# HummaWhite/ReSTIR

Hardware: AMD Instinct MI355X
Metric: Mrays/s (1920x1080 ReSTIR-DI, 32 candidates, spatiotemporal reuse) (higher is better)
Workload: dtype f32

## Files before the change

include/restir_hip.h:

```cpp
#ifndef RESTIR_HIP_H
#define RESTIR_HIP_H

#include <stdint.h>

#ifdef __cplusplus
extern "C" {
#endif

#define RS_ERR_INVALID_ARGUMENT 10001
#define RS_ERR_UNSUPPORTED      10002
#define RS_ERR_INTERNAL         10003

typedef struct rs_material {
    int   type;
    float baseColor[3];
    float metallic;
    float roughness;
    float ior;
    int   baseColorMapId;
    int   metallicMapId;
    int   roughnessMapId;
    int   normalMapId;
} rs_material;

// ... 264 lines not shown
    int tuneCounted;
    int tuneRestart;
    int stream;
    int lastChains;
    int splitSlot, splitCall, splitMode;
    int shadowOnLibrary;
    int risForm;
    int tilesX, tilesY, fusedTilesY;
    int cut;
} rs_phase_a_plan;
int  rs_debug_phase_a_plan(const rs_phase_a_inputs* in, rs_phase_a_plan* out);
int  rs_restir_set_primary_cuts(rs_restir* r, int on);
int  rs_debug_set_primary_cut_cap(rs_restir* r, int records);
int  rs_debug_primary_cut_info(rs_restir* r, int* cells, int* cellsWithoutCut, unsigned long long* records, int* usedLastFrame, unsigned long long* builds);
int  rs_debug_primary_cut_missing(rs_restir* r, const rs_scene* scene, int cell, int n, const float* rays, unsigned long long out[4]);
int  rs_restir_set_primary_leaf_lists(rs_restir* r, int on);
int  rs_debug_set_primary_leaf_list_cap(rs_restir* r, int records);
int  rs_debug_primary_leaf_list_info(rs_restir* r, int* tiles, int* tilesWithoutList, unsigned long long* records, int* usedLastFrame, unsigned long long* builds);
int  rs_debug_primary_leaf_list_missing(rs_restir* r, const rs_scene* scene, int n, const float* rays, unsigned long long out[4]);
int  rs_debug_plan_primary_leaf_list(const rs_camera* cam, int x0, int y0, int bvhSize, const float* boundingBoxes, const int* const bvhNodes[6], int cap,
                                     int* order, int* count, int* positions);
int  rs_debug_plan_primary_cut(const rs_camera* cam, int x0, int y0, int w, int h, int bvhSize, const float* boundingBoxes, const int* const bvhNodes[6], int cap,
                               int* order, int* count, int* positions, int* links);
typedef struct rs_primary_cut_key {
    unsigned long long sceneId, geomEdits;
    rs_camera cam;
    int y0, y1;
    unsigned cap, listCap;
} rs_primary_cut_key;
#define RS_CUT_ARENA_NOTHING   0
#define RS_CUT_ARENA_NO_MEMORY 1
#define RS_CUT_ARENA_BUILT     2
typedef struct rs_primary_cut_slot { int keyValid, cuts, lists; rs_primary_cut_key key; } rs_primary_cut_slot;
typedef struct rs_primary_cut_sizes { int numCells; unsigned capacity; int numTiles; unsigned listCapacity; } rs_primary_cut_sizes;
int  rs_debug_plan_primary_cut_slot(int on, int capturing, rs_primary_cut_slot* slot, const rs_primary_cut_key* key, int tilesX, int tilesY,
                                    int* cutState, rs_primary_cut_sizes* sizes);
#ifndef RS_AUX_STREAMS
#define RS_AUX_STREAMS 3
#endif
#define RS_STREAM_CHOICES_KEPT 4
#define RS_STREAMS_HELD_NONE     0
#define RS_STREAMS_HELD_MEASURED 1
#define RS_STREAMS_HELD_PLAIN    2
#define RS_STREAMS_PENDING_NONE         0
#define RS_STREAMS_PENDING_AGAIN        1
#define RS_STREAMS_PENDING_AGAIN_FORGET 2
// ... 148 lines not shown
```

restir_amd/capi.py:

```python
import ctypes as C
import os

import numpy as np

from .ctypes_structs import Camera, Material, Reservoir, MATERIAL_DTYPE, RESERVOIR_DTYPE, INDIRECT_RESERVOIR_DTYPE, LIGHT_SAMPLE_DTYPE, copy_camera
from .ctypes_structs import GeometryEditLights, GeometryEditPlan, GeometryEditView
from .ctypes_structs import STREAM_CHOICES_KEPT, StreamChoice, StreamChoiceInputs, StreamChoicePlan, StreamChoices

_HERE = os.path.dirname(os.path.abspath(__file__))
LIB_PATH = os.environ.get("RESTIR_HIP_LIB") or os.path.join(_HERE, "librestir_hip.so")


class RestirHipError(RuntimeError):
    pass


RS_ERR_INVALID_ARGUMENT, RS_ERR_UNSUPPORTED = 10001, 10002

TRANSPORT_GROUP = C.CFUNCTYPE(C.c_int, C.c_void_p)
TRANSPORT_SEND = C.CFUNCTYPE(C.c_int, C.c_void_p, C.c_void_p, C.c_size_t, C.c_int, C.c_void_p)
TRANSPORT_RECV = C.CFUNCTYPE(C.c_int, C.c_void_p, C.c_void_p, C.c_size_t, C.c_int, C.c_void_p)


class Transport(C.Structure):
# ... 97 lines not shown


class PrimaryCutSlot(C.Structure):
    _fields_ = [("keyValid", C.c_int), ("cuts", C.c_int), ("lists", C.c_int), ("key", PrimaryCutKey)]


class PrimaryCutSizes(C.Structure):
    _fields_ = [("numCells", C.c_int), ("capacity", C.c_uint), ("numTiles", C.c_int), ("listCapacity", C.c_uint)]


CUT_ARENA_NOTHING, CUT_ARENA_NO_MEMORY, CUT_ARENA_BUILT = 0, 1, 2
STREAMS_HELD_NONE, STREAMS_HELD_MEASURED, STREAMS_HELD_PLAIN = 0, 1, 2
STREAMS_PENDING_NONE, STREAMS_PENDING_AGAIN, STREAMS_PENDING_AGAIN_FORGET = 0, 1, 2


EXPORTS = [
    "rs_last_error", "rs_context_create", "rs_context_destroy", "rs_context_set_current", "rs_init", "rs_set_stream", "rs_set_sync", "rs_set_side_stream", "rs_set_ris_table_pixels", "rs_set_internal_stream_priority", "rs_internal_streams_info", "rs_choose_internal_streams_again", "rs_prepare_streams", "rs_set_stream_plan", "rs_set_denoise_stream", "rs_join_denoise_stream", "rs_set_tile_split", "rs_debug_split_tiles", "rs_synchronize",
    "rs_build_bvh", "rs_build_light_table", "rs_build_alias_table", "rs_build_envmap_pdf", "rs_scene_build", "rs_scene_build_textured", "rs_scene_create",
    "rs_scene_host_desc", "rs_scene_set_sample_sequence", "rs_scene_set_emission", "rs_scene_set_materials", "rs_scene_set_texture", "rs_scene_set_triangles", "rs_scene_set_geometry", "rs_scene_set_motion_tracking", "rs_scene_advance_motion", "rs_scene_download_prev_vertices", "rs_refit_boxes", "rs_debug_scene_table", "rs_debug_scene_grid", "rs_debug_scene_emissive_grid", "rs_debug_grid_box", "rs_scene_destroy", "rs_camera_update", "rs_trace_closest", "rs_trace_closest_wave", "rs_scene_set_ordered_tree", "rs_ordered_bvh_host_check", "rs_trace_occlusion",
    "rs_gbuffer_create", "rs_gbuffer_destroy", "rs_gbuffer_render", "rs_gbuffer_render_rows", "rs_gbuffer_update",
    "rs_gbuffer_get_view", "rs_gbuffer_set_reuse", "rs_gbuffer_reuse_stats", "rs_gbuffer_invalidate", "rs_gbuffer_rows_bytes", "rs_gbuffer_rows_pack", "rs_gbuffer_rows_unpack", "rs_restir_init", "rs_restir_free", "rs_restir_reset", "rs_restir_direct",
    "rs_restir_phase_a", "rs_restir_phase_b", "rs_restir_end_frame", "rs_restir_launch_choice", "rs_restir_halo_bytes", "rs_restir_halo_pack",
    "rs_restir_halo_unpack", "rs_restir_rows_bytes", "rs_restir_rows_pack", "rs_restir_rows_unpack", "rs_restir_download", "rs_restir_upload", "rs_restir_set_light_tracking", "rs_restir_download_light_ids", "rs_restir_set_light_retargeting", "rs_restir_get_light_retargeting", "rs_restir_download_light_samples", "rs_debug_restir_retarget", "rs_debug_restir_retarget_launched", "rs_debug_restir_surface_wo", "rs_scene_light_moves", "rs_restir_light_rows_bytes", "rs_restir_light_rows_pack", "rs_restir_light_rows_unpack", "rs_restir_ray_count", "rs_restir_ray_total", "rs_restir_pass_times",
    "rs_restir_enable_timing", "rs_restir_spatial_times", "rs_restir_set_probe", "rs_restir_last_launch", "rs_debug_phase_a_plan", "rs_restir_set_primary_cuts", "rs_debug_set_primary_cut_cap", "rs_debug_primary_cut_info", "rs_debug_primary_cut_missing", "rs_restir_set_primary_leaf_lists", "rs_debug_set_primary_leaf_list_cap", "rs_debug_primary_leaf_list_info", "rs_debug_primary_leaf_list_missing", "rs_debug_plan_primary_leaf_list", "rs_debug_plan_primary_cut", "rs_debug_plan_primary_cut_slot", "rs_debug_plan_stream_choice", "rs_debug_plan_stream_switch", "rs_debug_restir_surface", "rs_pbo_register", "rs_pbo_map", "rs_pbo_unmap", "rs_pbo_unregister", "rs_save_image", "rs_save_image_jpg", "rs_write_png", "rs_write_jpg", "rs_debug_tap_estimate_error", "rs_debug_sqrt_of_uniform_mismatches", "rs_debug_sqrt_of_unit_floats_mismatches", "rs_debug_exact_ops_mismatches", "rs_debug_rng_step_mismatches", "rs_debug_rng_step_host_mismatches", "rs_debug_div_sigma_mismatches", "rs_path_trace_init", "rs_path_trace_free", "rs_path_trace_direct",
    "rs_path_trace", "rs_path_trace_indirect", "rs_restir_indirect", "rs_restir_download_indirect",
    "rs_svgf_create", "rs_svgf_destroy", "rs_svgf_filter", "rs_svgf_next_frame", "rs_svgf_get_view",
    "rs_copy_image_to_pbo", "rs_copy_image2_to_pbo", "rs_copy_imagef_to_pbo", "rs_copy_imagei_to_pbo", "rs_eaw_create", "rs_eaw_destroy", "rs_eaw_set_params", "rs_eaw_get_params", "rs_eaw_set_tiled", "rs_eaw_set_fused", "rs_svgf_set_params", "rs_svgf_get_params", "rs_svgf_set_tiled", "rs_svgf_set_fused", "rs_eaw_filter", "rs_eaw_positions_rows", "rs_eaw_level_rows", "rs_modulate_albedo",
    "rs_add_image", "rs_add_image3", "rs_comm_create_rccl", "rs_comm_create_rccl_lib", "rs_comm_create", "rs_comm_destroy", "rs_comm_self_exchange", "rs_strips_create", "rs_strips_destroy", "rs_strips_rows", "rs_strips_set_comm_stream", "rs_strips_set_gbuffer_halo", "rs_strips_set_light_tracking", "rs_strips_frame", "rs_strips_eaw_filter", "rs_strips_svgf_filter", "rs_strips_exchange_svgf_history", "rs_strips_exchange_history", "rs_strips_gather", "rs_strips_gather_begin", "rs_strips_gather_end", "rs_strips_enable_timing", "rs_strips_halo_wait_ms",
    "rs_scene_file_load", "rs_scene_file_get", "rs_scene_file_free", "rs_build_transformation_matrix", "rs_bake_instance",
    "rs_bake_matrix", "rs_scene_file_objects", "rs_scene_define_parts", "rs_scene_set_part_transforms", "rs_scene_parts_info", "rs_scene_download_part_rest", "rs_debug_scene_staged_bytes", "rs_debug_plan_geometry_edit",
]

_lib = None


def lib():
    global _lib
    if _lib is not None:
        return _lib
    try:
        import torch
    except ImportError:
        pass
    if not os.path.exists(LIB_PATH):
        raise RestirHipError(
            f"{LIB_PATH} is missing: build it with `make -C restir_amd/csrc` (or __graft_entry__.build()). "
            "There is no CPU fallback for the MI355X path.")
# ... 81 lines not shown
    L.rs_restir_launch_choice.argtypes = [vp, C.POINTER(ci)]
    L.rs_restir_halo_bytes.argtypes = [vp, ci]
    L.rs_restir_halo_bytes.restype = C.c_size_t
    L.rs_restir_halo_pack.argtypes = [vp, ci, ci, vp]
    L.rs_restir_halo_unpack.argtypes = [vp, ci, ci, vp]
    L.rs_restir_rows_bytes.argtypes = [vp, ci, ci]
    L.rs_restir_rows_bytes.restype = C.c_size_t
    L.rs_debug_tap_estimate_error.argtypes = [ci, C.POINTER(cf)]
    L.rs_restir_last_launch.argtypes = [vp, C.POINTER(ci), C.POINTER(ci)]
    L.rs_debug_phase_a_plan.argtypes = [C.POINTER(PhaseAInputs), C.POINTER(PhaseAPlan)]
    L.rs_debug_plan_geometry_edit.argtypes = [C.POINTER(GeometryEditView), C.c_char_p, ci, ci, vp, vp, vp, ci, C.POINTER(GeometryEditPlan), vp,
                                              C.POINTER(GeometryEditLights), vp, vp, vp]
    L.rs_restir_set_primary_cuts.argtypes = [vp, ci]
    L.rs_debug_set_primary_cut_cap.argtypes = [vp, ci]
    L.rs_debug_primary_cut_info.argtypes = [vp, C.POINTER(ci), C.POINTER(ci), C.POINTER(C.c_ulonglong), C.POINTER(ci), C.POINTER(C.c_ulonglong)]
    L.rs_debug_primary_cut_missing.argtypes = [vp, vp, ci, ci, vp, C.POINTER(C.c_ulonglong * 4)]
    L.rs_restir_set_primary_leaf_lists.argtypes = [vp, ci]
    L.rs_debug_set_primary_leaf_list_cap.argtypes = [vp, ci]
    L.rs_debug_primary_leaf_list_info.argtypes = [vp, C.POINTER(ci), C.POINTER(ci), C.POINTER(C.c_ulonglong), C.POINTER(ci), C.POINTER(C.c_ulonglong)]
    L.rs_debug_primary_leaf_list_missing.argtypes = [vp, vp, ci, vp, C.POINTER(C.c_ulonglong * 4)]
    L.rs_debug_plan_primary_leaf_list.argtypes = [vp, ci, ci, ci, vp, C.POINTER(vp * 6), ci, C.POINTER(ci), C.POINTER(ci), vp]
    L.rs_debug_plan_primary_cut.argtypes = [vp, ci, ci, ci, ci, ci, vp, C.POINTER(vp * 6), ci, C.POINTER(ci), C.POINTER(ci), vp, vp]
    L.rs_debug_plan_primary_cut_slot.argtypes = [ci, ci, C.POINTER(PrimaryCutSlot), C.POINTER(PrimaryCutKey), ci, ci, C.POINTER(ci), C.POINTER(PrimaryCutSizes)]
    L.rs_debug_plan_stream_choice.argtypes = [C.POINTER(StreamChoiceInputs), C.POINTER(StreamChoicePlan)]
    L.rs_debug_plan_stream_switch.argtypes = [C.POINTER(StreamChoices), ci, vp, ci, C.POINTER(StreamChoice), C.POINTER(ci)]
    L.rs_debug_restir_surface.argtypes = [vp, vp, vp, vp]
    L.rs_pbo_register.argtypes = [C.c_uint, C.POINTER(vp)]
    L.rs_pbo_map.argtypes = [vp, C.POINTER(vp), C.POINTER(C.c_size_t)]
    L.rs_pbo_unmap.argtypes = [vp]
    L.rs_pbo_unregister.argtypes = [vp]
    L.rs_save_image.argtypes = [C.c_char_p, vp, ci, ci, ci]
    L.rs_write_png.argtypes = [C.c_char_p, vp, ci, ci]
    L.rs_write_jpg.argtypes = [C.c_char_p, vp, ci, ci]
    L.rs_svgf_set_tiled.argtypes = [vp, ci]
    L.rs_svgf_set_fused.argtypes = [vp, ci]
    L.rs_save_image_jpg.argtypes = [C.c_char_p, vp, ci, ci, ci]
    L.rs_debug_sqrt_of_uniform_mismatches.argtypes = [C.POINTER(C.c_ulonglong)]
    L.rs_debug_sqrt_of_unit_floats_mismatches.argtypes = [C.POINTER(C.c_ulonglong)]
    L.rs_debug_exact_ops_mismatches.argtypes = [ci, C.c_uint, C.c_uint, ci, ci, C.POINTER(C.c_ulonglong)]
    L.rs_debug_div_sigma_mismatches.argtypes = [C.c_float, C.POINTER(C.c_ulonglong)]
    L.rs_debug_rng_step_mismatches.argtypes = [C.POINTER(C.c_ulonglong * 2)]
    L.rs_debug_rng_step_host_mismatches.argtypes = [C.c_uint, C.c_uint, C.POINTER(C.c_ulonglong * 2)]
    L.rs_scene_set_sample_sequence.argtypes = [vp, vp, ci, ci]
    L.rs_set_stream_plan.argtypes = [ci, ci, ci]
    L.rs_set_denoise_stream.argtypes = [ci]
    L.rs_join_denoise_stream.argtypes = []
# ... 226 lines not shown
    order, count = C.c_int(), C.c_int()
    pos = np.zeros(max(int(cap), 1), np.int32)
    check(lib().rs_debug_plan_primary_leaf_list(C.byref(cam), int(x0), int(y0), nodes.shape[1], _p(boxes), C.byref(arr), int(cap), C.byref(order), C.byref(count), _p(pos)))
    return order.value, count.value, pos[:min(count.value, int(cap))].copy()


def plan_primary_cut(cam, x0, y0, w, h, boxes, nodes, cap):
    boxes = np.ascontiguousarray(boxes, np.float32); nodes = np.ascontiguousarray(nodes, np.int32)
    arr = (C.c_void_p * 6)(*[nodes[i].ctypes.data for i in range(6)])
    order, count = C.c_int(), C.c_int()
    pos, links = np.zeros(max(int(cap), 1), np.int32), np.zeros(max(int(cap), 1), np.int32)
    check(lib().rs_debug_plan_primary_cut(C.byref(cam), int(x0), int(y0), int(w), int(h), nodes.shape[1], _p(boxes), C.byref(arr), int(cap),
                                          C.byref(order), C.byref(count), _p(pos), _p(links)))
    kept = min(count.value, int(cap))
    return order.value, count.value, pos[:kept].copy(), links[:kept if count.value <= int(cap) else 0].copy()


def plan_primary_cut_slot(slot, key, on=True, capturing=False, tiles=(1, 1)):
    state, sizes = C.c_int(), PrimaryCutSizes()
    check(lib().rs_debug_plan_primary_cut_slot(int(on), int(capturing), C.byref(slot), C.byref(key), int(tiles[0]), int(tiles[1]), C.byref(state), C.byref(sizes)))
    return state.value, sizes


def plan_stream_choice(priority_range, asked=2, caller_priority=None, times_us=None):
    i, o = StreamChoiceInputs(), StreamChoicePlan()
    i.least, i.greatest, i.asked = int(priority_range[0]), int(priority_range[1]), int(asked)
    i.callerHasStream, i.callerPriority = int(caller_priority is not None), int(caller_priority or 0)
    for lvl in range(3):
        for k in range(4):
            i.timesUs[lvl][k] = 1.0 if times_us is None else float(times_us[lvl][k])
    check(lib().rs_debug_plan_stream_choice(C.byref(i), C.byref(o)))
    return o


def plan_stream_switch(state, caller, level_key=2, forget=False):
    released, n = (StreamChoice * (STREAM_CHOICES_KEPT + 1))(), C.c_int()
    check(lib().rs_debug_plan_stream_switch(C.byref(state), int(forget), C.c_void_p(caller), int(level_key), released, C.byref(n)))
    return [released[k] for k in range(n.value)]


def build_bvh(vertices):
    v = np.ascontiguousarray(vertices, np.float32).reshape(-1)
    n = v.size // 9
    size = 2 * n - 1
    boxes = np.zeros((size, 6), np.float32)
    nodes = np.zeros((6, size, 3), np.int32)
# ... 510 lines not shown
        return a.value, b.value

    def set_primary_cuts(self, on=True):
        check(lib().rs_restir_set_primary_cuts(self.handle, 1 if on else 0))

    def set_primary_cut_cap(self, records):
        check(lib().rs_debug_set_primary_cut_cap(self.handle, records))

    def primary_cut_info(self):
        a, b, u = C.c_int(), C.c_int(), C.c_int()
        n, k = C.c_ulonglong(), C.c_ulonglong()
        check(lib().rs_debug_primary_cut_info(self.handle, C.byref(a), C.byref(b), C.byref(n), C.byref(u), C.byref(k)))
        return dict(cells=a.value, without_cut=b.value, records=n.value, used=bool(u.value), builds=k.value)

    def primary_cut_missing(self, scene, cell, rays):
        rays = np.ascontiguousarray(rays, np.float32).reshape(-1, 4)
        out = (C.c_ulonglong * 4)()
        check(lib().rs_debug_primary_cut_missing(self.handle, scene.handle, cell, len(rays), _p(rays), C.byref(out)))
        return dict(missing=out[0], passed=out[1], left_out=out[2], records=out[3])

    def set_primary_leaf_lists(self, on=True):
        check(lib().rs_restir_set_primary_leaf_lists(self.handle, 1 if on else 0))

    def set_primary_leaf_list_cap(self, records):
        check(lib().rs_debug_set_primary_leaf_list_cap(self.handle, records))

    def primary_leaf_list_info(self):
        a, b, u = C.c_int(), C.c_int(), C.c_int()
        n, k = C.c_ulonglong(), C.c_ulonglong()
        check(lib().rs_debug_primary_leaf_list_info(self.handle, C.byref(a), C.byref(b), C.byref(n), C.byref(u), C.byref(k)))
        return dict(tiles=a.value, without_list=b.value, records=n.value, used=bool(u.value), builds=k.value)

    def primary_leaf_list_missing(self, scene, rays):
        rays = np.ascontiguousarray(rays, np.float32).reshape(-1, 4)
        out = (C.c_ulonglong * 4)()
        check(lib().rs_debug_primary_leaf_list_missing(self.handle, scene.handle, len(rays), _p(rays), C.byref(out)))
        return dict(missing=out[0], passed=out[1], left_out=out[2])

    def surface(self):
        n = self.width * self.height
        a, b, c = np.zeros((n, 4), np.float32), np.zeros((n, 4), np.float32), np.zeros((n, 2), np.uint32)
        check(lib().rs_debug_restir_surface(self.handle, _p(a), _p(b), _p(c)))
        return a, b, c

    def surface_wo(self):
        out = np.zeros((self.width * self.height, 4), np.float32)
# ... 350 lines not shown
```

restir_amd/csrc/restir.hip:

```cpp
#include <cstdlib>
#include <cstring>

#include "rs_row_layouts.h"
#include "rs_light_history.h"
#include "rs_cuts.h"

using namespace rs;

namespace {

constexpr int kReservoirSize = 32;
constexpr int kHalo = RS_SPATIAL_HALO_ROWS;

constexpr int kDrawsPrimary = 4, kDrawsRis = kDrawsPrimary + 5 * 32;
constexpr unsigned kTemporalDrewBit = 1u << 29;
constexpr int kRaySlots = 1024;
template <bool TEX>
__device__ __forceinline__ int primary_store(const DevScene& s, const SurfPlanes& sp, int index, const Ray& ray, const Hit& h, unsigned rngWord) {
    int shaded = 0;
    int kind = kKindMiss, matId = 0, type = 0;
    f3 norm = splat(0.f), wo = splat(0.f), p = h.pos;
    float metallic = 0.f, roughness = 0.f;
    if (h.primId != kNullPrim) {
        matId = h.matId;
        norm = h.norm;
        const SurfMat m = TEX ? textured_material(s, h, norm) : plain_material(s, matId);
        type = m.type; metallic = m.metallic; roughness = m.roughness;
        if (type == 4) {
// ... 251 lines not shown
__device__ __forceinline__ float ld_stream(const float* p) { return __builtin_nontemporal_load(p); }
__device__ __forceinline__ int ld_stream(const int* p) { return __builtin_nontemporal_load(p); }
__device__ __forceinline__ f3 ld3_stream(const float* p) { return mk3(__builtin_nontemporal_load(p), __builtin_nontemporal_load(p + 1), __builtin_nontemporal_load(p + 2)); }
__device__ __forceinline__ void st_stream(float4* p, float x, float y, float z, float w) { __builtin_nontemporal_store(vf4{ x, y, z, w }, reinterpret_cast<vf4*>(p)); }

__device__ __forceinline__ void resv_store(const ResvPlanes& p, int i, const Resv& r) {
    st_stream(p.li + i, r.Li.x, r.Li.y, r.Li.z, r.dist);
    st_stream(p.wi + i, r.wi.x, r.wi.y, r.wi.z, 0.f);
    __builtin_nontemporal_store(r.W, p.w + i);
    __builtin_nontemporal_store(r.M, p.m + i);
}

__global__ void __launch_bounds__(256, RS_WALK_WAVES) k_shadow(DevScene s, SurfPlanes sp, int width, int y0, int y1, int tilesX) {
    RS_SETPRIO(RS_PRIO_WALK);
    int x, y;
    pixel_of_lane(tilesX, y0, x, y);
    const bool inside = x < width && y < y1;
    const int index = inside ? y * width + x : 0;
    const float4 pm = inside ? sp.posMat[index] : make_float4(0.f, 0.f, 0.f, 0.f);
    const bool shaded = inside && mk_kind(__float_as_int(pm.w)) == kKindShaded;
    float4 cl = make_float4(0.f, 0.f, 0.f, 0.f), cw = cl;
    if (shaded) { cl = sp.candLi[index]; cw = sp.candWi[index]; }
    const f3 pos = mk3(pm.x, pm.y, pm.z), wi = mk3(cw.x, cw.y, cw.z);
    const bool occluded = trace_occluded_wave(s, pos, pos + wi * cl.w, shaded);
    if (shaded && occluded) reinterpret_cast<float*>(sp.candWi + index)[3] = 0.f;
}

template <bool SOBOL, int LIGHTS>
__device__ __forceinline__ void temporal_body(const SurfPlanes& sp, const GBufView& g, const ResvPlanes& last, const ResvPlanes& cur, const TempPlanes& temp, const uint32_t* sampleSeq, int looper,
                                              int first, int reuse, int n0, int n1, unsigned long long* rayWork, unsigned long long* rayDone, const LightIds& ids,
                                              const LightRecs& recs) {
    constexpr bool TRACK = LIGHTS >= 1, RETARGET = LIGHTS == 2;
    RS_SETPRIO(RS_PRIO_STREAM);
    if (blockIdx.x == 0 && threadIdx.x < kRaySub) {
        const int k = threadIdx.x * kRayStride;
        rayDone[k] = rayWork[k];
        rayWork[k] = 0;
    }
    const int index = n0 + blockIdx.x * blockDim.x + threadIdx.x;
    if (index >= n1) return;
    const uint2 rm = sp.rngMat[index];
    const bool shaded = mk_kind((int)rm.y) == kKindShaded;
    const int gid = ld_stream(g.primId + index);
    const float gdepth = ld_stream(g.depth + index);
    if (!shaded) {
        if (reuse & 2) {
            reinterpret_cast<float2*>(temp.tap + index)[1] = make_float2(__int_as_float(gid), gdepth);
            if (TRACK) {
// ... 406 lines not shown
    rs_dev_free(r->dRayCount);
    for (auto& perStream : r->split) for (auto& t : perStream) rs_tile_split_free(&t);
    rs_dev_free(r->indResv[0]); rs_dev_free(r->indResv[1]);
    rs_light_history_free(r->lights);
    rs_primary_cuts_destroy(r->cuts);
    for (auto& e : r->ev) if (e) (void)hipEventDestroy(e);
    for (auto& pair : r->spatialEv) for (hipEvent_t& e : pair) if (e) (void)hipEventDestroy(e);
    for (auto& e : r->surfFree) if (e) (void)hipEventDestroy(e);
    for (auto& e : r->tune.ev) if (e) (void)hipEventDestroy(e);
    if (r->auxFork) (void)hipEventDestroy(r->auxFork);
    if (r->auxDone) (void)hipEventDestroy(r->auxDone);
    delete r;
    return 0;
}

int rs_restir_init(int width, int height, rs_restir** out) {
    if (!out || width <= 0 || height <= 0) return rs_fail(RS_ERR_INVALID_ARGUMENT, "rs_restir_init: bad size");
    *out = nullptr;
    rs_restir* r = new rs_restir();
    r->ctx = rs_ctx();
    rs_ctx_scope scope(r->ctx);
    r->width = width; r->height = height;
    rs_primary_cuts_init(r->cuts);
    const size_t n = (size_t)width * height;
    int e = 0;
    if (!e) e = alloc_planes(r->cur, n);
    if (!e) e = alloc_planes(r->last, n);
    if (!e) e = rs_dev_alloc(&r->temp.li, n);
    if (!e) e = rs_dev_alloc(&r->temp.wi, n);
    if (!e) e = rs_dev_alloc(&r->temp.tap, n);
    if (!e) e = rs_check_hip(hipMemset(r->temp.li, 0, n * 16), "memset");
    if (!e) e = rs_check_hip(hipMemset(r->temp.wi, 0, n * 16), "memset");
    if (!e) e = rs_check_hip(hipMemset(r->temp.tap, 0, n * 16), "memset");
    for (auto& f : r->surf) {
        if (!e) e = rs_dev_alloc(&f.posKind, n);
        if (!e) e = rs_dev_alloc(&f.norm, n);
        if (!e) e = rs_dev_alloc(&f.wo, n);
        if (!e) e = rs_dev_alloc(&f.rngMat, n);
        if (!e) e = rs_dev_alloc(&f.candLi, n);
        if (!e) e = rs_dev_alloc(&f.candWi, n);
        if (!e) e = rs_check_hip(hipMemset(f.rngMat, 0, n * 8), "memset");
    }
    for (auto& ev : r->surfFree) if (!e) e = rs_check_hip(hipEventCreateWithFlags(&ev, hipEventDisableTiming), "hipEventCreate");
    for (auto& ev : r->tune.ev) if (!e) e = rs_check_hip(hipEventCreate(&ev), "hipEventCreate");
    if (!e) e = rs_check_hip(hipEventCreateWithFlags(&r->auxFork, hipEventDisableTiming), "hipEventCreate");
    if (!e) e = rs_check_hip(hipEventCreateWithFlags(&r->auxDone, hipEventDisableTiming), "hipEventCreate");
// ... 8 lines not shown

int rs_restir_reset(rs_restir* r) {
    RS_SCOPE(r);
    if (!r) return rs_fail(RS_ERR_INVALID_ARGUMENT, "rs_restir_reset: null");
    r->firstFrame = true;
    return 0;
}

int rs_restir_enable_timing(rs_restir* r, int enable) {
    RS_SCOPE(r);
    if (!r) return rs_fail(RS_ERR_INVALID_ARGUMENT, "rs_restir_enable_timing: null");
    r->timing = enable == 2 ? 2 : (enable != 0 ? 1 : 0);
    if (r->timing == 2) {
        for (auto& pair : r->spatialEv) for (hipEvent_t& e : pair) if (!e) RS_HIP(hipEventCreate(&e));
        r->spatialNext = 0;
    }
    return 0;
}

int rs_restir_set_probe(rs_restir* r, int enable) {
    RS_SCOPE(r);
    if (!r) return rs_fail(RS_ERR_INVALID_ARGUMENT, "rs_restir_set_probe: null");
    r->probe = enable != 0;
    return 0;
}

int rs_restir_spatial_times(rs_restir* r, float* ms, int capacity, int* count) {
    RS_SCOPE(r);
    if (!r || !ms || !count || capacity < 0) return rs_fail(RS_ERR_INVALID_ARGUMENT, "rs_restir_spatial_times: bad argument");
    *count = 0;
    if (r->timing != 2) return rs_fail(RS_ERR_INVALID_ARGUMENT, "rs_restir_spatial_times: rs_restir_enable_timing(r, 2) is not in force");
    RS_HIP(hipStreamSynchronize(rs_stream()));
    int n = r->spatialNext < rs_restir::kSpatialRing ? r->spatialNext : rs_restir::kSpatialRing;
    if (n > capacity) n = capacity;
    for (int i = 0; i < n; i++) {
        const int slot = (r->spatialNext - n + i) % rs_restir::kSpatialRing;
        RS_HIP(hipEventElapsedTime(&ms[i], r->spatialEv[slot][0], r->spatialEv[slot][1]));
    }
    *count = n;
    return 0;
}

}

namespace {
int launch_ris(const rs_scene* scene, const SurfPlanes& sp, int W, int y0, int y1, int looper, bool sobol, hipStream_t st, int form, const rs_light_history& lights, int set) {
    const int npx = (y1 - y0) * W;
    const dim3 grid((npx + kRisThreads - 1) / kRisThreads);
    static const bool ldsAllowed = []{
        bool ok = true;
        for (int mode = 0; mode < 3; mode++) rs_dispatch_lights(mode, [&](auto LIGHTS) {
            for (const void* k : { reinterpret_cast<const void*>(&k_ris_alias_lds<true, LIGHTS()>), reinterpret_cast<const void*>(&k_ris_alias_lds<false, LIGHTS()>) })
                ok = hipFuncSetAttribute(k, hipFuncAttributeMaxDynamicSharedMemorySize, kRisAliasLdsLights * (int)sizeof(AliasRec)) == hipSuccess && ok;
        });
        (void)hipGetLastError();
        return ok; }();
    (void)ldsAllowed;
    rs_dispatch_lights(rs_light_mode(lights), [&](auto LIGHTS) {
        const RisWinners<LIGHTS()> win = rs_light_history_winners<LIGHTS()>(lights, set);
        if (form == RS_RIS_LDS)
            rs_dispatch([&](auto SOBOL) { hipLaunchKernelGGL((k_ris_lds<SOBOL(), LIGHTS()>), grid, dim3(kRisThreads), 0, st, scene->dev, sp, W, y0, y1, looper, win); }, sobol);
        else if (form == RS_RIS_ALIAS_LDS)
            rs_dispatch([&](auto SOBOL) { hipLaunchKernelGGL((k_ris_alias_lds<SOBOL(), LIGHTS()>), grid, dim3(kRisThreads), (size_t)scene->numLights * sizeof(AliasRec), st, scene->dev, sp, W, y0, y1, looper, win); }, sobol);
        else
            rs_dispatch([&](auto ENV, auto SOBOL) { hipLaunchKernelGGL((k_ris<ENV(), SOBOL(), LIGHTS()>), dim3((npx + 255) / 256), dim3(256), 0, st, scene->dev, sp, W, y0, y1, looper, win); },
                        scene->envMapTexId >= 0, sobol);
    });
    return 0;
}

int phase_a_impl(rs_restir* r, const rs_scene* scene, const rs_camera* cam, const rs_gbuffer* g, int looper, int reuse, int y0, int y1, bool last) {
    RS_TRY(check_frame_args(r, scene, cam, g));
    RS_TRY(rs_check_looper(scene, looper, "ReSTIRDirect"));
    const bool sobol = scene->dev.sampleSeq != nullptr;
    r->looper = looper;
    if (y0 < 0) y0 = 0;
    if (y1 > r->height) y1 = r->height;
    r->raySlot = (r->raySlot + 1) % kRaySlots;
    unsigned long long* rayCounter = r->dRayCount + (size_t)r->raySlot * kRaySub * kRayStride;
    unsigned long long* rayDone = rayCounter + (size_t)kRaySlots * kRaySub * kRayStride;
    const rs_context* plan = rs_stream_plan();
    const rs_gbuffer::Deferred& d = g->deferred;
    static const bool reusedThree = [] { const char* e = std::getenv("RS_REUSE_CHAINS"); return !(e && std::atoi(e) == 2); }();
    const int W = r->width;
    rs_phase_a_inputs in{};
    in.async = r->timing != 1 && rs_aux_stream(1) != nullptr;
    in.chainStreams = plan->chainStreams; in.smallChains = plan->smallChains; in.shadowOnMain = plan->shadowOnMain;
    in.fuseMode = rs_fuse_mode();
    in.denoiseStream = rs_ctx()->denoiseMode == 1;
    in.chainsInFlight = rs_chains_in_flight();
    in.reusedThree = reusedThree;
// ... 52 lines not shown
        RS_TRY(rs_tile_split_prepare(hints, ((((long long)1 << 20 | d.y0) << 20 | d.y1) << 12 | tilesX) ^ ((long long)(y0 * 4099 + y1) << 44), tilesX * 4 * gTilesY, tilesX * gTilesY, p.splitMode, st, &ts, &helpers));
        rs_dispatch([&](auto TEX, auto SOBOL, auto MOTION) {
            if (ts.base) hipLaunchKernelGGL((k_gbuffer_primary_split<TEX(), SOBOL(), MOTION()>), dim3(helpers + tilesX * gTilesY), dim3(256), 0, st, scene->dev, cp, lp, gw, sp, looper, d.y0, d.y1, y0, y1, tilesX, rayCounter, ts);
            else hipLaunchKernelGGL((k_gbuffer_primary<TEX(), SOBOL(), MOTION()>), dim3(tilesX * gTilesY), dim3(256), 0, st, scene->dev, cp, lp, gw, sp, looper, d.y0, d.y1, y0, y1, tilesX, rayCounter);
        }, tex, sobol, scene->dev.prevVertices != nullptr);
        RS_HIP(hipEventRecord(g->doneEv, aux));
        g->pending = true;
    }
    else {
        TileSplit ts; int helpers = 0;
        RS_TRY(rs_tile_split_prepare(hints, (((long long)y0 << 20 | y1) << 12 | tilesX), tilesX * 4 * tilesY, tilesX * tilesY, p.splitMode, st, &ts, &helpers));
        PrimaryCuts cuts{};
        if (p.cut == 2) RS_TRY(rs_primary_cuts_view(r->cuts, st, &cuts));
        rs_dispatch([&](auto TEX, auto SOBOL) {
            if (ts.base) hipLaunchKernelGGL((k_primary_split<TEX(), SOBOL()>), dim3(helpers + tilesX * tilesY), dim3(256), 0, st, scene->dev, cp, sp, looper, y0, y1, tilesX, rayCounter, ts, cuts);
            else hipLaunchKernelGGL((k_primary<TEX(), SOBOL()>), dim3(tilesX * tilesY), dim3(256), 0, st, scene->dev, cp, sp, looper, y0, y1, tilesX, rayCounter, cuts);
        }, tex, sobol);
        if (p.cut == 2) RS_TRY(rs_primary_cuts_launched(r->cuts, aux ? 1 + p.stream : 0, st));
    }
    mark(r, 1);
    const int npx = (y1 - y0) * W;
    RS_TRY(launch_ris(scene, sp, W, y0, y1, looper, sobol, st, p.risForm, r->lights, r->surfSet));
    mark(r, 2);
    if (!p.shadowOnLibrary) hipLaunchKernelGGL(k_shadow, dim3(tilesX * tilesY), dim3(256), 0, st, scene->dev, sp, W, y0, y1, tilesX);
    if (aux) {
        RS_TRY(rs_check_hip(hipGetLastError(), "ReSTIR Direct (primary / RIS / shadow rays)"));
        RS_HIP(hipEventRecord(r->auxDone, aux));
        RS_HIP(hipStreamWaitEvent(rs_stream(), r->auxDone, 0));
    }
    if (p.cut == 1) RS_TRY(rs_primary_cuts_build(r->cuts, scene, cp, y0, tilesX, tilesY, st));
    if (p.shadowOnLibrary) hipLaunchKernelGGL(k_shadow, dim3(tilesX * tilesY), dim3(256), 0, rs_stream(), scene->dev, sp, W, y0, y1, tilesX);
    RS_TRY(rs_gbuffer_join(g));
    LightIds ids; LightRecs recs;
    RS_TRY(rs_light_history_phase_a(r->lights, scene, r->surfSet, !r->firstFrame && (reuse & 1), sp, gbuf_view(g), r->last, y0, y1, tilesX, tilesY, rayCounter, &ids, &recs));
    rs_dispatch_lights(rs_light_mode(r->lights), [&](auto LIGHTS) {
        rs_dispatch([&](auto SOBOL) {
            hipLaunchKernelGGL((k_temporal<SOBOL(), LIGHTS()>), dim3((npx + 255) / 256), dim3(256), 0, rs_stream(), sp, gbuf_view(g), r->last, r->cur, r->temp,
                               scene->dev.sampleSeq, looper, r->firstFrame ? 1 : 0, reuse, y0 * W, y1 * W, rayCounter, rayDone, merge_lights<LIGHTS()>(ids, recs));
        }, sobol);
    });
    mark(r, 3);
    return last ? rs_after_launch("ReSTIR Direct (phase A)") : rs_check_hip(hipGetLastError(), "ReSTIR Direct (phase A)");
}

int phase_b_impl(rs_restir* r, const rs_scene* scene, const rs_camera* cam, const rs_gbuffer* g,
                 float* devDirectIllum, int iter, int reuse, int y0, int y1, bool last) {
    RS_TRY(check_frame_args(r, scene, cam, g));
    if (!devDirectIllum) return rs_fail(RS_ERR_INVALID_ARGUMENT, "ReSTIRDirect: null radiance buffer");
    if (y0 < 0) y0 = 0;
    if (y1 > r->height) y1 = r->height;
    if (y1 <= y0) return 0;
    const int tilesX = (r->width + kBTileW - 1) / kBTileW, tilesY = (y1 - y0 + kBTileH - 1) / kBTileH;
    const int numTiles = tilesX * tilesY;
    RS_TRY(rs_gbuffer_join(g));
// ... 44 lines not shown
    RS_SCOPE(r);
    return phase_b_impl(r, scene, cam, g, devDirectIllum, iter, reuse, y0, y1, true);
}

int rs_restir_last_launch(const rs_restir* r, int* fused, int* chains) {
    RS_SCOPE(r);
    if (!r || !fused || !chains) return rs_fail(RS_ERR_INVALID_ARGUMENT, "rs_restir_last_launch: null argument");
    *fused = r->lastFused; *chains = r->lastChains;
    return 0;
}

int rs_debug_restir_surface(rs_restir* r, float* posTag, float* normal, unsigned* rngTag) {
    RS_SCOPE(r);
    if (!r || !posTag || !normal || !rngTag) return rs_fail(RS_ERR_INVALID_ARGUMENT, "rs_debug_restir_surface: null argument");
    RS_TRY(rs_synchronize());
    const rs_restir::Surf& f = r->surf[(r->surfSet + rs_restir::kSurfSets - 1) % rs_restir::kSurfSets];
    const size_t n = (size_t)r->width * r->height;
    RS_HIP(hipMemcpy(posTag, f.posKind, n * 16, hipMemcpyDeviceToHost));
    RS_HIP(hipMemcpy(normal, f.norm, n * 16, hipMemcpyDeviceToHost));
    RS_HIP(hipMemcpy(rngTag, f.rngMat, n * 8, hipMemcpyDeviceToHost));
    return 0;
}

int rs_debug_restir_surface_wo(rs_restir* r, float* wo4) {
    RS_SCOPE(r);
    if (!r || !wo4) return rs_fail(RS_ERR_INVALID_ARGUMENT, "rs_debug_restir_surface_wo: null argument");
    RS_TRY(rs_synchronize());
    const rs_restir::Surf& f = r->surf[(r->surfSet + rs_restir::kSurfSets - 1) % rs_restir::kSurfSets];
    RS_HIP(hipMemcpy(wo4, f.wo, (size_t)r->width * r->height * 16, hipMemcpyDeviceToHost));
    return 0;
}

int rs_debug_phase_a_plan(const rs_phase_a_inputs* in, rs_phase_a_plan* out) {
    if (!in || !out) return rs_fail(RS_ERR_INVALID_ARGUMENT, "rs_debug_phase_a_plan: null argument");
    rs_plan_phase_a(*in, *out);
    return 0;
}

int rs_restir_launch_choice(const rs_restir* r, int* choice) {
    RS_SCOPE(r);
    if (!r || !choice) return rs_fail(RS_ERR_INVALID_ARGUMENT, "rs_restir_launch_choice: null argument");
    *choice = r->tune.reported();
    return 0;
}

int rs_restir_end_frame(rs_restir* r) {
// ... 207 lines not shown
```

restir_amd/csrc/rs_internal.h:

```cpp
#pragma once

#include <hip/hip_runtime.h>

#include <string>
#include <type_traits>
#ifndef RS_AUX_STREAMS
#define RS_AUX_STREAMS 3
#endif
#ifndef RS_SPLIT_SMALL_ROUNDS
#define RS_SPLIT_SMALL_ROUNDS 3
#endif
#include "rs_frame_plan.h"
#include "rs_cut_plan.h"
#include "rs_stream_choice.h"
#ifndef RS_GBUF_SETS
#define RS_GBUF_SETS (RS_AUX_STREAMS + 2)
#endif
#ifndef RS_SURF_SETS
#define RS_SURF_SETS (RS_AUX_STREAMS + 1)
#endif
#include <vector>

#include "rs_scene.h"
#include "rs_geometry_plan.h"
// ... 438 lines not shown
        uint2*  rngMat = nullptr;
        float4* candLi = nullptr;
        float4* candWi = nullptr;
    } surf[kSurfSets];
    int surfSet = 0, chain = 0, smallChain = 0;
    hipEvent_t surfFree[kSurfSets] = {};
    bool surfFreeValid[kSurfSets] = {};
    hipEvent_t auxFork = nullptr, auxDone = nullptr;
    int phaseACalls = 0;
    bool idleFrame = false;
    int idleStreak = 0;
    rs_fuse_tuner tune;
    int lastFused = -1, lastChains = 0;
    unsigned long long* dRayCount = nullptr;
    rs_tile_split split[1 + rs_context::kAux][3];
    int raySlot = 0;
    int timing = 0;
    hipEvent_t ev[5] = { nullptr, nullptr, nullptr, nullptr, nullptr };
    static constexpr int kSpatialRing = 256;
    hipEvent_t spatialEv[kSpatialRing][2] = {};
    int spatialNext = 0;
    bool probe = false;
    rs_light_history lights;
};

static_assert(rs_context::kAux >= 1 + rs_restir::kChains, "one auxiliary stream for GBuffer::render and one per chain");
static_assert(kPlanSmallChains == rs_context::kAux, "the plan's three chains are the context's auxiliary streams");

struct rs_eaw {
    rs_context* ctx = nullptr;
    int width = 0, height = 0, level = 0;
    float sigLumin = 64.f, sigNormal = .2f, sigDepth = 1.f;
    float* devTempImg = nullptr;
    float* devPos = nullptr;
    bool tiled = true;
    bool fused = true;
};

struct rs_svgf {
    rs_context* ctx = nullptr;
    int width = 0, height = 0, level = 0;
    float sigLumin = 4.f, sigNormal = 128.f, sigDepth = 1.f;
    float* devAccumColor[2] = { nullptr, nullptr };
    float* devAccumMoment[2] = { nullptr, nullptr };
    float* devVariance = nullptr;
    float* devTempColor = nullptr;
// ... 33 lines not shown
```

Before: 8276.

## Regroup shadow rays by length within each block before tracing occlusion

Adds a shadow-ray kernel that bins each tile's active shadow rays by length (relative to the scene extent) using a shared-memory histogram and prefix scan. Rays are compacted into LDS sorted longest-first, and each wave traces a coherent batch. Waves with no active rays exit early. The old kernel also now skips rays whose candidate weight is already zero. This targets wave divergence and idle lanes in the BVH occlusion walk, at the cost of extra LDS traffic, block-wide barriers and a scattered write-back of results. The feature is on by default.

```diff
diff --git a/include/restir_hip.h b/include/restir_hip.h
--- a/include/restir_hip.h
+++ b/include/restir_hip.h
@@ -310,6 +310,11 @@
                                      int* order, int* count, int* positions);
 int  rs_debug_plan_primary_cut(const rs_camera* cam, int x0, int y0, int w, int h, int bvhSize, const float* boundingBoxes, const int* const bvhNodes[6], int cap,
                                int* order, int* count, int* positions, int* links);
+int  rs_restir_set_shadow_regroup(rs_restir* r, int on);
+int  rs_debug_plan_shadow_regroup(int n, const float* lengths, const unsigned char* active, float binsOverExtent, const float* rootLo, const float* rootHi,
+                                  int* bins, int* first, int* count, float* binsOverExtentOut);
+int  rs_debug_shadow_pass(rs_restir* r, const rs_scene* scene, int y0, int y1, const float* posTag, const float* candLi, float* candWi, int* slots,
+                          float* binsOverExtent);
 typedef struct rs_primary_cut_key {
     unsigned long long sceneId, geomEdits;
     rs_camera cam;
diff --git a/restir_amd/capi.py b/restir_amd/capi.py
--- a/restir_amd/capi.py
+++ b/restir_amd/capi.py
@@ -143,7 +143,7 @@
     "rs_gbuffer_get_view", "rs_gbuffer_set_reuse", "rs_gbuffer_reuse_stats", "rs_gbuffer_invalidate", "rs_gbuffer_rows_bytes", "rs_gbuffer_rows_pack", "rs_gbuffer_rows_unpack", "rs_restir_init", "rs_restir_free", "rs_restir_reset", "rs_restir_direct",
     "rs_restir_phase_a", "rs_restir_phase_b", "rs_restir_end_frame", "rs_restir_launch_choice", "rs_restir_halo_bytes", "rs_restir_halo_pack",
     "rs_restir_halo_unpack", "rs_restir_rows_bytes", "rs_restir_rows_pack", "rs_restir_rows_unpack", "rs_restir_download", "rs_restir_upload", "rs_restir_set_light_tracking", "rs_restir_download_light_ids", "rs_restir_set_light_retargeting", "rs_restir_get_light_retargeting", "rs_restir_download_light_samples", "rs_debug_restir_retarget", "rs_debug_restir_retarget_launched", "rs_debug_restir_surface_wo", "rs_scene_light_moves", "rs_restir_light_rows_bytes", "rs_restir_light_rows_pack", "rs_restir_light_rows_unpack", "rs_restir_ray_count", "rs_restir_ray_total", "rs_restir_pass_times",
-    "rs_restir_enable_timing", "rs_restir_spatial_times", "rs_restir_set_probe", "rs_restir_last_launch", "rs_debug_phase_a_plan", "rs_restir_set_primary_cuts", "rs_debug_set_primary_cut_cap", "rs_debug_primary_cut_info", "rs_debug_primary_cut_missing", "rs_restir_set_primary_leaf_lists", "rs_debug_set_primary_leaf_list_cap", "rs_debug_primary_leaf_list_info", "rs_debug_primary_leaf_list_missing", "rs_debug_plan_primary_leaf_list", "rs_debug_plan_primary_cut", "rs_debug_plan_primary_cut_slot", "rs_debug_plan_stream_choice", "rs_debug_plan_stream_switch", "rs_debug_restir_surface", "rs_pbo_register", "rs_pbo_map", "rs_pbo_unmap", "rs_pbo_unregister", "rs_save_image", "rs_save_image_jpg", "rs_write_png", "rs_write_jpg", "rs_debug_tap_estimate_error", "rs_debug_sqrt_of_uniform_mismatches", "rs_debug_sqrt_of_unit_floats_mismatches", "rs_debug_exact_ops_mismatches", "rs_debug_rng_step_mismatches", "rs_debug_rng_step_host_mismatches", "rs_debug_div_sigma_mismatches", "rs_path_trace_init", "rs_path_trace_free", "rs_path_trace_direct",
+    "rs_restir_enable_timing", "rs_restir_spatial_times", "rs_restir_set_probe", "rs_restir_last_launch", "rs_debug_phase_a_plan", "rs_restir_set_primary_cuts", "rs_debug_set_primary_cut_cap", "rs_debug_primary_cut_info", "rs_debug_primary_cut_missing", "rs_restir_set_primary_leaf_lists", "rs_debug_set_primary_leaf_list_cap", "rs_debug_primary_leaf_list_info", "rs_debug_primary_leaf_list_missing", "rs_debug_plan_primary_leaf_list", "rs_debug_plan_primary_cut", "rs_debug_plan_primary_cut_slot", "rs_restir_set_shadow_regroup", "rs_debug_plan_shadow_regroup", "rs_debug_shadow_pass", "rs_debug_plan_stream_choice", "rs_debug_plan_stream_switch", "rs_debug_restir_surface", "rs_pbo_register", "rs_pbo_map", "rs_pbo_unmap", "rs_pbo_unregister", "rs_save_image", "rs_save_image_jpg", "rs_write_png", "rs_write_jpg", "rs_debug_tap_estimate_error", "rs_debug_sqrt_of_uniform_mismatches", "rs_debug_sqrt_of_unit_floats_mismatches", "rs_debug_exact_ops_mismatches", "rs_debug_rng_step_mismatches", "rs_debug_rng_step_host_mismatches", "rs_debug_div_sigma_mismatches", "rs_path_trace_init", "rs_path_trace_free", "rs_path_trace_direct",
     "rs_path_trace", "rs_path_trace_indirect", "rs_restir_indirect", "rs_restir_download_indirect",
     "rs_svgf_create", "rs_svgf_destroy", "rs_svgf_filter", "rs_svgf_next_frame", "rs_svgf_get_view",
     "rs_copy_image_to_pbo", "rs_copy_image2_to_pbo", "rs_copy_imagef_to_pbo", "rs_copy_imagei_to_pbo", "rs_eaw_create", "rs_eaw_destroy", "rs_eaw_set_params", "rs_eaw_get_params", "rs_eaw_set_tiled", "rs_eaw_set_fused", "rs_svgf_set_params", "rs_svgf_get_params", "rs_svgf_set_tiled", "rs_svgf_set_fused", "rs_eaw_filter", "rs_eaw_positions_rows", "rs_eaw_level_rows", "rs_modulate_albedo",
@@ -271,6 +271,10 @@
     L.rs_debug_plan_primary_leaf_list.argtypes = [vp, ci, ci, ci, vp, C.POINTER(vp * 6), ci, C.POINTER(ci), C.POINTER(ci), vp]
     L.rs_debug_plan_primary_cut.argtypes = [vp, ci, ci, ci, ci, ci, vp, C.POINTER(vp * 6), ci, C.POINTER(ci), C.POINTER(ci), vp, vp]
     L.rs_debug_plan_primary_cut_slot.argtypes = [ci, ci, C.POINTER(PrimaryCutSlot), C.POINTER(PrimaryCutKey), ci, ci, C.POINTER(ci), C.POINTER(PrimaryCutSizes)]
+    if hasattr(L, "rs_restir_set_shadow_regroup"):
+        L.rs_restir_set_shadow_regroup.argtypes = [vp, ci]
+        L.rs_debug_plan_shadow_regroup.argtypes = [ci, vp, vp, C.c_float, vp, vp, vp, vp, C.POINTER(ci), C.POINTER(C.c_float)]
+        L.rs_debug_shadow_pass.argtypes = [vp, vp, ci, ci, vp, vp, vp, vp, C.POINTER(C.c_float)]
     L.rs_debug_plan_stream_choice.argtypes = [C.POINTER(StreamChoiceInputs), C.POINTER(StreamChoicePlan)]
     L.rs_debug_plan_stream_switch.argtypes = [C.POINTER(StreamChoices), ci, vp, ci, C.POINTER(StreamChoice), C.POINTER(ci)]
     L.rs_debug_restir_surface.argtypes = [vp, vp, vp, vp]
@@ -543,6 +547,17 @@
     return state.value, sizes
 
 
+def plan_shadow_regroup(lengths, bins_over_extent=None, root=None, active=None, plan=False):
+    lengths = np.ascontiguousarray(lengths, np.float32).reshape(-1)
+    n = len(lengths)
+    bins, first, count, used = np.zeros(max(n, 1), np.int32), np.zeros(64, np.int32), C.c_int(), C.c_float()
+    act = None if active is None else np.ascontiguousarray(np.asarray(active) != 0, np.uint8)
+    lo, hi = (None, None) if root is None else (np.ascontiguousarray(root[0], np.float32), np.ascontiguousarray(root[1], np.float32))
+    check(lib().rs_debug_plan_shadow_regroup(n, _p(lengths), None if act is None else _p(act), float(bins_over_extent or 0.0), None if lo is None else _p(lo),
+                                             None if hi is None else _p(hi), _p(bins), _p(first) if plan else None, C.byref(count) if plan else None, C.byref(used)))
+    return (bins[:n], used.value, first, count.value) if plan else (bins[:n], used.value)
+
+
 def plan_stream_choice(priority_range, asked=2, caller_priority=None, times_us=None):
     i, o = StreamChoiceInputs(), StreamChoicePlan()
     i.least, i.greatest, i.asked = int(priority_range[0]), int(priority_range[1]), int(asked)
@@ -1099,6 +1114,17 @@
     def set_primary_leaf_lists(self, on=True):
         check(lib().rs_restir_set_primary_leaf_lists(self.handle, 1 if on else 0))
 
+    def set_shadow_regroup(self, on=True):
+        check(lib().rs_restir_set_shadow_regroup(self.handle, 1 if on else 0))
+
+    def shadow_pass(self, scene, pos_tag, cand_li, cand_wi, rows=None):
+        n = self.width * self.height
+        y0, y1 = rows or (0, self.height)
+        a, b = np.ascontiguousarray(pos_tag, np.float32).reshape(n, 4), np.ascontiguousarray(cand_li, np.float32).reshape(n, 4)
+        w, slots, k = np.array(cand_wi, np.float32).reshape(n, 4).copy(), np.zeros(n, np.int32), C.c_float()
+        check(lib().rs_debug_shadow_pass(self.handle, scene.handle, y0, y1, _p(a), _p(b), _p(w), _p(slots), C.byref(k)))
+        return w, slots, k.value
+
     def set_primary_leaf_list_cap(self, records):
         check(lib().rs_debug_set_primary_leaf_list_cap(self.handle, records))
 
diff --git a/restir_amd/csrc/restir.hip b/restir_amd/csrc/restir.hip
--- a/restir_amd/csrc/restir.hip
+++ b/restir_amd/csrc/restir.hip
@@ -4,6 +4,7 @@
 #include "rs_row_layouts.h"
 #include "rs_light_history.h"
 #include "rs_cuts.h"
+#include "rs_shadow_regroup.h"
 
 using namespace rs;
 
@@ -301,8 +302,48 @@
     float4 cl = make_float4(0.f, 0.f, 0.f, 0.f), cw = cl;
     if (shaded) { cl = sp.candLi[index]; cw = sp.candWi[index]; }
     const f3 pos = mk3(pm.x, pm.y, pm.z), wi = mk3(cw.x, cw.y, cw.z);
-    const bool occluded = trace_occluded_wave(s, pos, pos + wi * cl.w, shaded);
-    if (shaded && occluded) reinterpret_cast<float*>(sp.candWi + index)[3] = 0.f;
+    const bool walks = shaded && __float_as_uint(cw.w) != 0u;
+    const bool occluded = trace_occluded_wave(s, pos, pos + wi * cl.w, walks);
+    if (walks && occluded) reinterpret_cast<float*>(sp.candWi + index)[3] = 0.f;
+}
+
+__global__ void __launch_bounds__(kShadowRegroupRays, RS_WALK_WAVES) k_shadow_regroup(DevScene s, SurfPlanes sp, int width, int y0, int y1, int tilesX, float binsOverExtent, int* slotsOut) {
+    __shared__ float4 sRay[2 * kShadowRegroupRays];
+    __shared__ int sHist[kShadowBins];
+    RS_SETPRIO(RS_PRIO_WALK);
+    int x, y;
+    const int lane = pixel_of_lane(tilesX, y0, x, y);
+    if (threadIdx.x < kShadowBins) sHist[threadIdx.x] = 0;
+    const bool inside = x < width && y < y1;
+    const int index = inside ? y * width + x : 0;
+    const float4 pm = inside ? sp.posMat[index] : make_float4(0.f, 0.f, 0.f, 0.f);
+    const bool shaded = inside && mk_kind(__float_as_int(pm.w)) == kKindShaded;
+    float4 cl = make_float4(0.f, 0.f, 0.f, 0.f), cw = cl;
+    if (shaded) { cl = sp.candLi[index]; cw = sp.candWi[index]; }
+    const bool walks = shaded && __float_as_uint(cw.w) != 0u;
+    const int bin = shadow_bin(cl.w, binsOverExtent);
+    __syncthreads();
+    int rank = 0;
+    if (walks) rank = atomicAdd(&sHist[bin], 1);
+    __syncthreads();
+    int above = sHist[kShadowBins - 1 - lane];
+    for (int off = 1; off < 64; off <<= 1) { const int v = __shfl_up(above, off); above += lane >= off ? v : 0; }
+    const int count = __shfl(above, 63);
+    const int first = __shfl(above, bin < kShadowBins - 1 ? kShadowBins - 2 - bin : 0);
+    const int slot = (bin < kShadowBins - 1 ? first : 0) + rank;
+    if (walks) {
+        sRay[slot] = make_float4(pm.x, pm.y, pm.z, __int_as_float(index));
+        sRay[kShadowRegroupRays + slot] = make_float4(cw.x, cw.y, cw.z, cl.w);
+    }
+    if (slotsOut && inside) slotsOut[index] = walks ? slot : -1;
+    __syncthreads();
+    if ((int)(threadIdx.x & ~63u) >= count) return;
+    const bool mine = (int)threadIdx.x < count;
+    float4 a = make_float4(0.f, 0.f, 0.f, 0.f), b = a;
+    if (mine) { a = sRay[threadIdx.x]; b = sRay[kShadowRegroupRays + threadIdx.x]; }
+    const f3 pos = mk3(a.x, a.y, a.z), wi = mk3(b.x, b.y, b.z);
+    const bool occluded = trace_occluded_wave(s, pos, pos + wi * b.w, mine);
+    if (mine && occluded) reinterpret_cast<float*>(sp.candWi + __float_as_int(a.w))[3] = 0.f;
 }
 
 template <bool SOBOL, int LIGHTS>
@@ -755,6 +796,7 @@
     rs_ctx_scope scope(r->ctx);
     r->width = width; r->height = height;
     rs_primary_cuts_init(r->cuts);
+    if (const char* env = std::getenv("RS_SHADOW_REGROUP")) r->shadowRegroup = std::atoi(env) != 0;
     const size_t n = (size_t)width * height;
     int e = 0;
     if (!e) e = alloc_planes(r->cur, n);
@@ -809,6 +851,28 @@
     RS_SCOPE(r);
     if (!r) return rs_fail(RS_ERR_INVALID_ARGUMENT, "rs_restir_set_probe: null");
     r->probe = enable != 0;
+    return 0;
+}
+
+int rs_restir_set_shadow_regroup(rs_restir* r, int on) {
+    RS_SCOPE(r);
+    if (!r) return rs_fail(RS_ERR_INVALID_ARGUMENT, "rs_restir_set_shadow_regroup: null");
+    r->shadowRegroup = on != 0;
+    return 0;
+}
+
+int rs_debug_plan_shadow_regroup(int n, const float* lengths, const unsigned char* active, float binsOverExtent, const float* rootLo, const float* rootHi,
+                                 int* bins, int* first, int* count, float* binsOverExtentOut) {
+    if (n < 0 || (n > 0 && (!lengths || !bins)) || (!rootLo != !rootHi) || (!first != !count) || (first && n > kShadowRegroupRays))
+        return rs_fail(RS_ERR_INVALID_ARGUMENT, "rs_debug_plan_shadow_regroup: bad argument");
+    if (rootLo) binsOverExtent = shadow_bins_over_extent(rootLo, rootHi);
+    if (binsOverExtentOut) *binsOverExtentOut = binsOverExtent;
+    for (int i = 0; i < n; i++) bins[i] = shadow_bin(lengths[i], binsOverExtent);
+    if (first) {
+        int lanes[kShadowRegroupRays];
+        for (int i = 0; i < n; i++) lanes[i] = (!active || active[i]) ? bins[i] : -1;
+        *count = rs_plan_shadow_slots(lanes, n, first);
+    }
     return 0;
 }
 
@@ -854,6 +918,18 @@
                         scene->envMapTexId >= 0, sobol);
     });
     return 0;
+}
+
+float shadow_scale(const rs_scene* scene) {
+    const float lo[3] = { scene->dev.occRootLo.x, scene->dev.occRootLo.y, scene->dev.occRootLo.z }, hi[3] = { scene->dev.occRootHi.x, scene->dev.occRootHi.y, scene->dev.occRootHi.z };
+    return shadow_bins_over_extent(lo, hi);
+}
+
+void launch_shadow(const rs_restir* r, const rs_scene* scene, const SurfPlanes& sp, int W, int y0, int y1, int tilesX, int tilesY, hipStream_t st, int* slotsOut = nullptr) {
+    if (r->shadowRegroup && scene->dev.occNodes) {
+        hipLaunchKernelGGL(k_shadow_regroup, dim3(tilesX * tilesY), dim3(kShadowRegroupRays), 0, st, scene->dev, sp, W, y0, y1, tilesX, shadow_scale(scene), slotsOut);
+    }
+    else hipLaunchKernelGGL(k_shadow, dim3(tilesX * tilesY), dim3(256), 0, st, scene->dev, sp, W, y0, y1, tilesX);
 }
 
 int phase_a_impl(rs_restir* r, const rs_scene* scene, const rs_camera* cam, const rs_gbuffer* g, int looper, int reuse, int y0, int y1, bool last) {
@@ -952,14 +1028,14 @@
     const int npx = (y1 - y0) * W;
     RS_TRY(launch_ris(scene, sp, W, y0, y1, looper, sobol, st, p.risForm, r->lights, r->surfSet));
     mark(r, 2);
-    if (!p.shadowOnLibrary) hipLaunchKernelGGL(k_shadow, dim3(tilesX * tilesY), dim3(256), 0, st, scene->dev, sp, W, y0, y1, tilesX);
+    if (!p.shadowOnLibrary) launch_shadow(r, scene, sp, W, y0, y1, tilesX, tilesY, st);
     if (aux) {
         RS_TRY(rs_check_hip(hipGetLastError(), "ReSTIR Direct (primary / RIS / shadow rays)"));
         RS_HIP(hipEventRecord(r->auxDone, aux));
         RS_HIP(hipStreamWaitEvent(rs_stream(), r->auxDone, 0));
     }
     if (p.cut == 1) RS_TRY(rs_primary_cuts_build(r->cuts, scene, cp, y0, tilesX, tilesY, st));
-    if (p.shadowOnLibrary) hipLaunchKernelGGL(k_shadow, dim3(tilesX * tilesY), dim3(256), 0, rs_stream(), scene->dev, sp, W, y0, y1, tilesX);
+    if (p.shadowOnLibrary) launch_shadow(r, scene, sp, W, y0, y1, tilesX, tilesY, rs_stream());
     RS_TRY(rs_gbuffer_join(g));
     LightIds ids; LightRecs recs;
     RS_TRY(rs_light_history_phase_a(r->lights, scene, r->surfSet, !r->firstFrame && (reuse & 1), sp, gbuf_view(g), r->last, y0, y1, tilesX, tilesY, rayCounter, &ids, &recs));
@@ -1050,6 +1126,34 @@
     return 0;
 }
 
+int rs_debug_shadow_pass(rs_restir* r, const rs_scene* scene, int y0, int y1, const float* posTag, const float* candLi, float* candWi, int* slots, float* binsOverExtent) {
+    RS_SCOPE(r);
+    if (!r || !scene || !posTag || !candLi || !candWi || y0 < 0 || y1 > r->height || y1 <= y0) return rs_fail(RS_ERR_INVALID_ARGUMENT, "rs_debug_shadow_pass: bad argument");
+    if (scene->ctx != r->ctx) return rs_fail(RS_ERR_INVALID_ARGUMENT, "rs_debug_shadow_pass: the scene belongs to another context");
+    RS_TRY(rs_synchronize());
+    if (binsOverExtent) *binsOverExtent = scene->dev.occNodes ? shadow_scale(scene) : 0.f;
+    const size_t n = (size_t)r->width * r->height;
+    SurfPlanes sp{};
+    int* dSlots = nullptr;
+    int e = rs_dev_alloc(&sp.posMat, n);
+    if (!e) e = rs_dev_alloc(&sp.candLi, n);
+    if (!e) e = rs_dev_alloc(&sp.candWi, n);
+    if (!e) e = rs_dev_alloc(&dSlots, n);
+    if (!e) e = rs_check_hip(hipMemcpy(sp.posMat, posTag, n * 16, hipMemcpyHostToDevice), "rs_debug_shadow_pass");
+    if (!e) e = rs_check_hip(hipMemcpy(sp.candLi, candLi, n * 16, hipMemcpyHostToDevice), "rs_debug_shadow_pass");
+    if (!e) e = rs_check_hip(hipMemcpy(sp.candWi, candWi, n * 16, hipMemcpyHostToDevice), "rs_debug_shadow_pass");
+    if (!e) e = rs_check_hip(hipMemset(dSlots, 0xff, n * sizeof(int)), "rs_debug_shadow_pass");
+    if (!e) {
+        launch_shadow(r, scene, sp, r->width, y0, y1, (r->width + 31) / 32, (y1 - y0 + 7) / 8, rs_stream(), dSlots);
+        e = rs_after_launch("rs_debug_shadow_pass");
+    }
+    if (!e) e = rs_synchronize();
+    if (!e) e = rs_check_hip(hipMemcpy(candWi, sp.candWi, n * 16, hipMemcpyDeviceToHost), "rs_debug_shadow_pass");
+    if (!e && slots) e = rs_check_hip(hipMemcpy(slots, dSlots, n * sizeof(int), hipMemcpyDeviceToHost), "rs_debug_shadow_pass");
+    rs_dev_free(sp.posMat); rs_dev_free(sp.candLi); rs_dev_free(sp.candWi); rs_dev_free(dSlots);
+    return e;
+}
+
 int rs_debug_restir_surface_wo(rs_restir* r, float* wo4) {
     RS_SCOPE(r);
     if (!r || !wo4) return rs_fail(RS_ERR_INVALID_ARGUMENT, "rs_debug_restir_surface_wo: null argument");
diff --git a/restir_amd/csrc/rs_internal.h b/restir_amd/csrc/rs_internal.h
--- a/restir_amd/csrc/rs_internal.h
+++ b/restir_amd/csrc/rs_internal.h
@@ -484,6 +484,7 @@
     int spatialNext = 0;
     bool probe = false;
     rs_light_history lights;
+    bool shadowRegroup = true;
 };
 
 static_assert(rs_context::kAux >= 1 + rs_restir::kChains, "one auxiliary stream for GBuffer::render and one per chain");
diff --git a/restir_amd/csrc/rs_shadow_regroup.h b/restir_amd/csrc/rs_shadow_regroup.h
--- /dev/null
+++ b/restir_amd/csrc/rs_shadow_regroup.h
@@ -0,0 +1,29 @@
+#pragma once
+
+#if defined(__HIPCC__)
+#define RS_REGROUP_HD __host__ __device__ inline
+#else
+#define RS_REGROUP_HD inline
+#endif
+
+constexpr int kShadowBins = 64;
+constexpr int kShadowRegroupRays = 256;
+
+RS_REGROUP_HD int shadow_bin(float length, float binsOverExtent) {
+    const float t = length * binsOverExtent;
+    if (!(t < (float)(kShadowBins - 1))) return kShadowBins - 1;
+    return t > 0.f ? (int)t : 0;
+}
+
+inline float shadow_bins_over_extent(const float lo[3], const float hi[3]) {
+    const float dx = hi[0] - lo[0], dy = hi[1] - lo[1], dz = hi[2] - lo[2];
+    return (float)kShadowBins / __builtin_sqrtf(dx * dx + dy * dy + dz * dz);
+}
+
+inline int rs_plan_shadow_slots(const int* bins, int n, int first[kShadowBins]) {
+    int hist[kShadowBins] = {};
+    for (int i = 0; i < n; i++) if (bins[i] >= 0) hist[bins[i] < kShadowBins ? bins[i] : kShadowBins - 1]++;
+    int at = 0;
+    for (int b = kShadowBins - 1; b >= 0; b--) { first[b] = at; at += hist[b]; }
+    return at;
+}
```

Result: faster. 8565 (median of 6 runs) (+3.5%).
